# lsp-plugins/lsp-dsp-units

Measured on AMD Instinct MI355X. Metric: Msamples/sec per GPU (biquad-x8 1024ch; Convolver 65536-tap) + HBM roofline %, higher is better.
Workload: dtype f32; 1 GPU; biquad-x8 cascade (FilterBank::process), 1024 channels x 4096-sample blocks per GPU, FLT_BT_LRX_LOPASS slope 4 per-channel cutoffs, state carried across blocks; channels_per_gpu=1024, block=4096, resident_ring_blocks=16, parallelism=channel-shard x1, no collective, blocks_per_call=1657

## Files before the change

### lsp-dsp-units_amd/csrc/biquad.hip

```cpp
#include "mi_common.h"
#include "ilufs_device.h"

#include <algorithm>
#include <atomic>
#include <cmath>
#include <cstdint>
#include <cstdlib>
#include <vector>

namespace
{
    template <int L>
    struct geom
    {
        static constexpr int W      = 2 * L;
        static constexpr int TAB    = 96 + 2 * L;
        static constexpr int PITCH  = W + 4;
        static constexpr int BLOCK  = 64 * W;
        static constexpr int SG     = 128;
        static_assert(((PITCH / 4) & 1) == 1, "LDS pitch must be an odd number of 16-B slots");
        static_assert((TAB % 16) == 0, "table rows stay 64-B aligned (s_load_dwordx16)");
    };

    constexpr int TAB_PQ = 32;
    typedef float v2f  __attribute__((ext_vector_type(2)));
    typedef float v8f  __attribute__((ext_vector_type(8)));
    typedef float v16f __attribute__((ext_vector_type(16)));

    __device__ __forceinline__ v2f pk_fma(v2f a, v2f b, v2f c) { return __builtin_elementwise_fma(a, b, c); }
    __device__ __forceinline__ v2f splat(float a) { return v2f{a, a}; }
    __device__ __forceinline__ v2f mat_fma(v2f c0, v2f c1, v2f v, v2f a) { return pk_fma(c0, splat(v.x), pk_fma(c1, splat(v.y), a)); }

    template <int CTRL, int ROW_MASK>
    __device__ __forceinline__ float dpp_or(float old, float v)
    {
        return __int_as_float(__builtin_amdgcn_update_dpp(__float_as_int(old), __float_as_int(v), CTRL, ROW_MASK, 0xf, false));
    }
    template <int CTRL, int ROW_MASK>
    __device__ __forceinline__ v2f dpp_or(v2f old, v2f v) { return v2f{dpp_or<CTRL, ROW_MASK>(old.x, v.x), dpp_or<CTRL, ROW_MASK>(old.y, v.y)}; }

    template <int CTRL>
    __device__ __forceinline__ v2f dpp_zero(v2f v)
    {
        return v2f{__int_as_float(__builtin_amdgcn_update_dpp(0, __float_as_int(v.x), CTRL, 0xf, 0xf, true)),
                   __int_as_float(__builtin_amdgcn_update_dpp(0, __float_as_int(v.y), CTRL, 0xf, 0xf, true))};
    }

    constexpr int DPP_ROW_SHR1 = 0x111, DPP_ROW_SHR2 = 0x112, DPP_ROW_SHR4 = 0x114, DPP_ROW_SHR8 = 0x118;
    constexpr int DPP_WAVE_SHR1 = 0x138, DPP_ROW_BCAST15 = 0x142, DPP_ROW_BCAST31 = 0x143;

    using mi::BUFFER_DWORD3;
    using mi::CPOL_SC1;
    using mi::u32x4;
    using mi::CPOL_NT_SC1;
    template <int POL = CPOL_NT_SC1>
    __device__ __forceinline__ void store_through(__amdgpu_buffer_rsrc_t rsrc, int dword_index, float4 v)
    {
        mi::wt_store<POL>(rsrc, dword_index * 4, v);
    }

#ifndef MI_ABLATE
#define MI_ABLATE 0
#endif
#ifdef MI_BIQUAD_PROBE
    __device__ unsigned long long g_probe[4096 * 16 * 2];
    #define MI_PROBE(slot) do { __builtin_amdgcn_sched_barrier(0); if (t == 0 && (slot) < 16) { \
        const unsigned pw_ = blockIdx.x * (blockDim.x >> 6) + (threadIdx.x >> 6); \
        g_probe[(pw_ * 16 + (slot)) * 2] = wall_clock64(); \
        g_probe[(pw_ * 16 + (slot)) * 2 + 1] = __builtin_readcyclecounter(); } __builtin_amdgcn_sched_barrier(0); } while (0)
#else
    #define MI_PROBE(slot) do { } while (0)
#endif
    constexpr int CHAIN_MAX = 14;
    struct chain_stage
    {
        const float    *tab;
        float          *state;
        const uint32_t *nsec;
        float          *out;
        size_t          out_stride;
        int             max_sec;
        int             branch;
    };
    struct chain_args
// ... 83 lines not shown
        {
            for (int i = tid; i < group; i += NT)
                sstate[par][lds0 + i] = reinterpret_cast<const float2 *>(mem + size_t(s0) * 2)[i];
        };
        auto flush_state = [&](float *mem, int s0, int group, int par, int lds0)
        {
            for (int i = tid; i < group; i += NT)
                reinterpret_cast<float2 *>(mem + size_t(s0) * 2)[i] = sstate[par][lds0 + i];
        };

        v2f x[L];

        struct sectab
        {
            v16f pq[L / 8];
            v8f  m0;
            v16f m1;
            float4 cf;
            float  a2;
            float4 ql;
        };
        typedef const __attribute__((address_space(4))) float cfloat;
        auto uniform_row = [&](const float *T) -> cfloat * {
            const uint64_t v = reinterpret_cast<uint64_t>(T);
            const uint32_t lo = uint32_t(__builtin_amdgcn_readfirstlane(int(uint32_t(v))));
            const uint32_t hi = uint32_t(__builtin_amdgcn_readfirstlane(int(uint32_t(v >> 32))));
            return reinterpret_cast<cfloat *>((uint64_t(hi) << 32) | lo);
        };
        typedef const __attribute__((address_space(4))) v16f cv16f;
        typedef const __attribute__((address_space(4))) v8f cv8f;
        auto load_pq = [&](sectab &r, const float *T)
        {
            cfloat *U = uniform_row(T);
            #pragma unroll
            for (int j = 0; j < L / 8; ++j)
                r.pq[j] = *reinterpret_cast<cv16f *>(U + TAB_PQ + 16 * j);
        };
        auto load_mats = [&](sectab &r, const float *T)
        {
            cfloat *U = uniform_row(T);
            r.m0 = *reinterpret_cast<cv8f *>(U + 8);
            r.m1 = *reinterpret_cast<cv16f *>(U + 16);
            r.ql = *reinterpret_cast<const float4 *>(T + TAB_QL + 4 * l16);
        };
        auto load_coefs = [&](sectab &r, const float *T)
        {
            cfloat *U = uniform_row(T);
            r.cf = make_float4(U[0], U[1], U[2], U[3]);
            r.a2 = U[4];
        };

        auto section = [&](sectab &tb, const float *Tnext, int si, int par, bool saver, bool save_hi)
        {
            v2f a0 = splat(0.0f), a1_ = splat(0.0f), b0_ = splat(0.0f), b1_ = splat(0.0f);
            #pragma unroll
            for (int k = 0; k < L; k += 2)
            {
                const v16f &r = tb.pq[k / 8];
                const v2f pq0 = v2f{r[(2 * k) % 16], r[(2 * k + 1) % 16]};
                const v2f pq1 = v2f{r[(2 * k + 2) % 16], r[(2 * k + 3) % 16]};
                a0  = pk_fma(pq0, splat(x[k].x), a0);      b0_ = pk_fma(pq0, splat(x[k].y), b0_);
                a1_ = pk_fma(pq1, splat(x[k + 1].x), a1_); b1_ = pk_fma(pq1, splat(x[k + 1].y), b1_);
            }
            const v2f zwA = a0 + a1_, zwB = b0_ + b1_;

            const v2f Pc0 = v2f{tb.m0[0], tb.m0[1]}, Pc1 = v2f{tb.m0[2], tb.m0[3]};
            v2f e = mat_fma(Pc0, Pc1, zwA, zwB);

            if (XW > 1)
                for (int v = 0; v < wv; ++v)
                    __syncthreads();
            const float2 cs = (XW > 1 && wv > 0) ? xchg[par][si][wv - 1] : sstate[par][si];
            const v2f cvec = lane0 ? v2f{cs.x, cs.y} : splat(0.0f);
            e = mat_fma(v2f{tb.m0[4], tb.m0[5]}, v2f{tb.m0[6], tb.m0[7]}, cvec, e);

            const v2f zero = splat(0.0f);
            e = mat_fma(v2f{tb.m0[4], tb.m0[5]}, v2f{tb.m0[6], tb.m0[7]}, dpp_zero<DPP_ROW_SHR1>(e), e);
            e = mat_fma(v2f{tb.m1[0], tb.m1[1]}, v2f{tb.m1[2], tb.m1[3]}, dpp_zero<DPP_ROW_SHR2>(e), e);
            e = mat_fma(v2f{tb.m1[4], tb.m1[5]}, v2f{tb.m1[6], tb.m1[7]}, dpp_zero<DPP_ROW_SHR4>(e), e);
            e = mat_fma(v2f{tb.m1[8], tb.m1[9]}, v2f{tb.m1[10], tb.m1[11]}, dpp_zero<DPP_ROW_SHR8>(e), e);
            const v2f QLc0 = v2f{tb.ql.x, tb.ql.y}, QLc1 = v2f{tb.ql.z, tb.ql.w};
            e = mat_fma(QLc0, QLc1, dpp_or<DPP_ROW_BCAST15, 0xa>(zero, e), e);
            {
                const v2f s  = dpp_or<DPP_ROW_BCAST31, 0xc>(zero, e);
                const v2f s2 = mat_fma(v2f{tb.m1[12], tb.m1[13]}, v2f{tb.m1[14], tb.m1[15]}, s, zero);
                e = mat_fma(QLc0, QLc1, row3 ? s2 : s, e);
            }
            if (XW > 1)
            {
                if (t == 63)
                    xchg[par][si][wv] = make_float2(e.x, e.y);
                for (int v = wv; v < XW - 1; ++v)
                    __syncthreads();
            }

            const v2f S  = dpp_or<DPP_WAVE_SHR1, 0xf>(cvec, e);
            const v2f SB = mat_fma(Pc0, Pc1, S, zwA);
            v2f d0 = v2f{S.x, SB.x}, d1 = v2f{S.y, SB.y};
            __builtin_amdgcn_sched_barrier(0);
            load_pq(tb, Tnext);
            load_mats(tb, Tnext);
            __builtin_amdgcn_sched_barrier(0);

            const v2f b0 = splat(tb.cf.x), b1 = splat(tb.cf.y), b2 = splat(tb.cf.z), a1 = splat(tb.cf.w), a2 = splat(tb.a2);
            #pragma unroll
            for (int k = 0; k < L; ++k)
            {
                const v2f xx = x[k];
                const v2f tq = pk_fma(b1, xx, d1);
                const v2f u  = b2 * xx;
                const v2f y  = pk_fma(b0, xx, d0);
                d0   = pk_fma(a1, y, tq);
                d1   = pk_fma(a2, y, u);
                x[k] = y;
            }
            __builtin_amdgcn_sched_barrier(0);
            load_coefs(tb, Tnext);
// ... 348 lines not shown

#ifdef MI_BIQUAD_PROBE
    #define MI_STREAM_PROBE_BEGIN() unsigned long long pc_[4] = {0, 0, 0, 0}, pt_ = __builtin_readcyclecounter(), pw0_ = wall_clock64(), \
        pw1_ = 0, pw2_ = 0; const unsigned long long pc0_ = pt_; unsigned spins_ = 0
    #define MI_STREAM_PROBE(slot) do { __builtin_amdgcn_sched_barrier(0); const unsigned long long now_ = __builtin_readcyclecounter(); \
        pc_[slot] += now_ - pt_; pt_ = now_; if ((slot) == 1 && pw1_ == 0) pw1_ = wall_clock64(); if ((slot) == 3 && pw2_ == 0) pw2_ = wall_clock64(); \
        __builtin_amdgcn_sched_barrier(0); } while (0)
    #define MI_STREAM_PROBE_SPIN() (++spins_)
    #define MI_STREAM_PROBE_ITER(it) do { if (t == 0 && (it) < 20) g_probe[(size_t(blockIdx.x) * NW + wv) * 32 + 11 + (it)] = \
        (wall_clock64() & 0xffffffffull) | ((__builtin_readcyclecounter() & 0xffffffffull) << 32); } while (0)
    #define MI_STREAM_PROBE_END() do { if (t == 0) { unsigned long long *p_ = g_probe + (size_t(blockIdx.x) * NW + wv) * 32; \
        p_[0] = pw0_; p_[1] = wall_clock64(); p_[2] = __builtin_readcyclecounter() - pc0_; p_[3] = pc_[1]; p_[4] = pc_[2]; p_[5] = pc_[3] + pc_[0]; \
        p_[6] = spins_; p_[7] = pw1_; p_[8] = pw2_; \
        p_[9] = __builtin_amdgcn_s_getreg((31 << 11) | 4); p_[10] = __builtin_amdgcn_s_getreg((31 << 11) | 20); } } while (0)
#else
    #define MI_STREAM_PROBE_BEGIN() do { } while (0)
    #define MI_STREAM_PROBE(slot) do { } while (0)
    #define MI_STREAM_PROBE_SPIN() do { } while (0)
    #define MI_STREAM_PROBE_ITER(it) do { } while (0)
    #define MI_STREAM_PROBE_END() do { } while (0)
#endif
#ifndef MI_STREAM_ROTATE
#define MI_STREAM_ROTATE 1
#endif
    constexpr int STREAM_MAX_BLOCKS = 128;
    constexpr int STREAM_SG         = 32;
    struct stream_args
    {
        int             blocks;
        float          *out[STREAM_MAX_BLOCKS];
        const float    *in[STREAM_MAX_BLOCKS];
    };
    constexpr int STREAM_CHAIN_BLOCKS = 64;
    constexpr int STREAM_CHAIN_PTRS   = 320;
    struct stream_chain_stage
    {
        const float    *tab;
        float          *state;
        const uint32_t *nsec;
        int             max_sec;
        int             slot;
        int             branch;
    };
    struct stream_chain_args
    {
        int                 blocks, stages, outs;
        stream_chain_stage  st[CHAIN_MAX];
        const float        *in[STREAM_CHAIN_BLOCKS];
        float              *out[STREAM_CHAIN_PTRS];
    };
    struct stream_cell { float d0, d1; uint32_t seq, pad; };
    typedef volatile __attribute__((address_space(3))) stream_cell lds_cell;

    template <int NW, bool CHAIN, bool QLDS>
    __device__ __forceinline__
    void biquad_stream_body(const stream_args *pa, const stream_chain_args *pc, size_t out_stride, size_t in_stride,
                            int n , const float *__restrict__ tab, float *state,
                            const uint32_t *__restrict__ nsec, int max_sec, int cap)
    {
        using G = geom<16>;
        constexpr int L = 16, W = G::W, TAB = G::TAB, PITCH = G::PITCH, SB = G::BLOCK;
        constexpr int LPT = W / 4;
        constexpr int TAB_QL = TAB_PQ + 2 * L;
        __shared__ __attribute__((aligned(16))) float sx_all[NW * 64 * PITCH];
        extern __shared__ float4 stream_dyn[];
        stream_cell *const cell = reinterpret_cast<stream_cell *>(stream_dyn);
        const float4 *const sql = stream_dyn + cap * NW;

        const int ch  = int(blockIdx.x);
        const int tid = int(threadIdx.x);
        const int t   = tid & 63;
        const int wv  = __builtin_amdgcn_readfirstlane(tid >> 6);
        const int l16 = t & 15;
        float *const sx = sx_all + wv * 64 * PITCH;
        const bool lane0 = (t == 0), row3 = (t >= 48);
        const int nst = CHAIN ? pc->stages : 1;
        auto stage_ns  = [&](int k) -> int { return CHAIN ? int(pc->st[k].nsec[ch]) : int(nsec[ch]); };
        auto stage_tab = [&](int k) -> const float * {
            return CHAIN ? pc->st[k].tab + size_t(ch) * pc->st[k].max_sec * TAB : tab + size_t(ch) * max_sec * TAB; };
        auto stage_mem = [&](int k) -> float * {
            return CHAIN ? pc->st[k].state + size_t(ch) * pc->st[k].max_sec * 2 : state + size_t(ch) * max_sec * 2; };
        const float *ctab = stage_tab(0);
        float2 *const mem0 = reinterpret_cast<float2 *>(stage_mem(0));
        const int spb   = (n + SB - 1) / SB;
        const int total = (CHAIN ? pc->blocks : pa->blocks) * spb;
        const int pred  = (wv + NW - 1) % NW;

        typedef const __attribute__((address_space(4))) float cfloat;
        typedef const __attribute__((address_space(4))) v16f cv16f;
        typedef const __attribute__((address_space(4))) v8f cv8f;
        auto uniform_row = [&](const float *T) -> cfloat * {
            const uint64_t v = reinterpret_cast<uint64_t>(T);
            const uint32_t lo = uint32_t(__builtin_amdgcn_readfirstlane(int(uint32_t(v))));
            const uint32_t hi = uint32_t(__builtin_amdgcn_readfirstlane(int(uint32_t(v >> 32))));
            return reinterpret_cast<cfloat *>((uint64_t(hi) << 32) | lo);
        };
        struct sectab
        {
            v16f pq[L / 8];
            v8f  m0;
            v16f m1;
            float4 cf;
            float  a2;
            float4 ql;
        };
        auto load_pq = [&](sectab &r, const float *T)
        {
            cfloat *U = uniform_row(T);
            #pragma unroll
            for (int j = 0; j < L / 8; ++j)
                r.pq[j] = *reinterpret_cast<cv16f *>(U + TAB_PQ + 16 * j);
        };
        auto load_mats = [&](sectab &r, const float *T, int qi )
        {
            cfloat *U = uniform_row(T);
            r.m0 = *reinterpret_cast<cv8f *>(U + 8);
            r.m1 = *reinterpret_cast<cv16f *>(U + 16);
            r.ql = QLDS ? sql[qi * 16 + l16] : *reinterpret_cast<const float4 *>(T + TAB_QL + 4 * l16);
        };
        auto load_coefs = [&](sectab &r, const float *T)
        {
            cfloat *U = uniform_row(T);
            r.cf = make_float4(U[0], U[1], U[2], U[3]);
            r.a2 = U[4];
        };

        float4 ld[LPT];
        auto issue_loads = [&](int g, bool there = true)
        {
            const int k = g / spb, j = g - k * spb;
            const float *blk = CHAIN ? pc->in[k] : pa->in[k];
            const __amdgpu_buffer_rsrc_t src = __builtin_amdgcn_make_buffer_rsrc(
                const_cast<float *>(blk + size_t(ch) * in_stride), 0, there ? n * 4 : 0, BUFFER_DWORD3);
            #pragma unroll
            for (int q = 0; q < LPT; ++q)
            {
                const u32x4 v = __builtin_amdgcn_raw_buffer_load_b128(src, (j * SB + 4 * (q * 64 + t)) * 4, 0, 0);
                ld[q] = make_float4(__uint_as_float(v.x), __uint_as_float(v.y), __uint_as_float(v.z), __uint_as_float(v.w));
            }
        };

        if (wv < total)
            issue_loads(wv);
        if (QLDS)
        {
            const __amdgpu_buffer_rsrc_t none = __builtin_amdgcn_make_buffer_rsrc(state, 0, 0, BUFFER_DWORD3);
            #pragma unroll
            for (int q = 0; q < LPT; ++q)
                store_through(none, 4 * (q * 64 + t), make_float4(0.0f, 0.0f, 0.0f, 0.0f));
        }
        const int ns  = stage_ns(0);
        if (!CHAIN && ns < 0)
            return;
        {
            int lds0 = 0;
            for (int k = 0; k < nst; ++k)
            {
                const int nk = (k == 0) ? ns : stage_ns(k);
                const float *mk = stage_mem(k);
                for (int i = tid; i < nk * NW; i += 64 * NW)
                {
                    const int si = i / NW, w = i - si * NW;
                    stream_cell c = { 0.0f, 0.0f, 0u, 0u };
                    if (w == NW - 1)
                    {
                        const float2 s = reinterpret_cast<const float2 *>(mk)[si];
                        c.d0 = s.x;
                        c.d1 = s.y;
                    }
                    cell[(lds0 + si) * NW + w] = c;
                }
                if (QLDS)
                {
                    const float *tk = stage_tab(k);
                    for (int i = tid; i < nk * 16; i += 64 * NW)
                        stream_dyn[cap * NW + lds0 * 16 + i] = *reinterpret_cast<const float4 *>(tk + size_t(i >> 4) * TAB + TAB_QL + 4 * (i & 15));
                }
                lds0 += nk;
            }
        }
        __syncthreads();

        v2f x[L];
        sectab tb;
        if (CHAIN || ns > 0)
        {
            load_pq(tb, ctab);
            load_mats(tb, ctab, 0);
            load_coefs(tb, ctab);
        }
        MI_STREAM_PROBE_BEGIN();

        for (int g = wv; g < total; g += NW)
        {
            MI_STREAM_PROBE(0);
            const int k = g / spb, j = g - k * spb;
            const int base  = j * SB;
            const int valid = (n - base < SB) ? n - base : SB;
            const int last  = valid - 1;
            const int t_last = last / W;
            const bool save_hi = (last - t_last * W) >= L;
            const bool saver   = (t == t_last);
            const bool exact_out = (j & 1) || (j == spb - 1);
            const bool final_sb  = (g == total - 1);
            const uint32_t want = uint32_t(g), mine = uint32_t(g + 1);

            #pragma unroll
            for (int q = 0; q < LPT; ++q)
            {
                const int i = 4 * (q * 64 + t);
                float *d = &sx[(i / W) * PITCH + 2 * (i % L) + ((i % W) / L)];
                d[0] = ld[q].x; d[2] = ld[q].y; d[4] = ld[q].z; d[6] = ld[q].w;
            }
            __builtin_amdgcn_wave_barrier();
            MI_STREAM_PROBE(1);
            if (!CHAIN && g + NW < total)
                issue_loads(g + NW);
            #pragma unroll
            for (int q = 0; q < L / 2; ++q)
            {
                const float4 v = *reinterpret_cast<const float4 *>(&sx[t * PITCH + 4 * q]);
                x[2 * q] = v2f{v.x, v.y};
                x[2 * q + 1] = v2f{v.z, v.w};
            }

            auto section = [&](const float *Tnext, int qnext, int ci, float2 *mem2, int turn)
            {
#if MI_STREAM_ROTATE
                if ((turn & 3) == 0)
                    switch (((turn >> 2) + (g / NW) + int(blockIdx.x >> 8)) & 3)
                    {
                        case 0: __builtin_amdgcn_s_setprio(3); break;
                        case 1: __builtin_amdgcn_s_setprio(2); break;
                        case 2: __builtin_amdgcn_s_setprio(1); break;
                        default: __builtin_amdgcn_s_setprio(0); break;
                    }
#endif
                lds_cell *const from = (lds_cell *)&cell[ci * NW + pred];
                lds_cell *const to   = (lds_cell *)&cell[ci * NW + wv];
                uint32_t got = from->seq;
                float c0 = from->d0, c1 = from->d1;

                v2f a0 = splat(0.0f), a1_ = splat(0.0f), b0_ = splat(0.0f), b1_ = splat(0.0f);
                #pragma unroll
                for (int q = 0; q < L; q += 2)
                {
                    const v16f &r = tb.pq[q / 8];
                    const v2f pq0 = v2f{r[(2 * q) % 16], r[(2 * q + 1) % 16]};
                    const v2f pq1 = v2f{r[(2 * q + 2) % 16], r[(2 * q + 3) % 16]};
                    a0  = pk_fma(pq0, splat(x[q].x), a0);      b0_ = pk_fma(pq0, splat(x[q].y), b0_);
                    a1_ = pk_fma(pq1, splat(x[q + 1].x), a1_); b1_ = pk_fma(pq1, splat(x[q + 1].y), b1_);
                }
                const v2f zwA = a0 + a1_, zwB = b0_ + b1_;

                const v2f Pc0 = v2f{tb.m0[0], tb.m0[1]}, Pc1 = v2f{tb.m0[2], tb.m0[3]};
                v2f e = mat_fma(Pc0, Pc1, zwA, zwB);
                asm volatile("" : "+v"(e));
                while (got != want)
                {
                    MI_STREAM_PROBE_SPIN();
                    __builtin_amdgcn_s_sleep(1);
                    got = from->seq;
                    c0 = from->d0;
                    c1 = from->d1;
                }
                const v2f cvec = lane0 ? v2f{c0, c1} : splat(0.0f);
                e = mat_fma(v2f{tb.m0[4], tb.m0[5]}, v2f{tb.m0[6], tb.m0[7]}, cvec, e);

                const v2f zero = splat(0.0f);
                e = mat_fma(v2f{tb.m0[4], tb.m0[5]}, v2f{tb.m0[6], tb.m0[7]}, dpp_zero<DPP_ROW_SHR1>(e), e);
                e = mat_fma(v2f{tb.m1[0], tb.m1[1]}, v2f{tb.m1[2], tb.m1[3]}, dpp_zero<DPP_ROW_SHR2>(e), e);
                e = mat_fma(v2f{tb.m1[4], tb.m1[5]}, v2f{tb.m1[6], tb.m1[7]}, dpp_zero<DPP_ROW_SHR4>(e), e);
                e = mat_fma(v2f{tb.m1[8], tb.m1[9]}, v2f{tb.m1[10], tb.m1[11]}, dpp_zero<DPP_ROW_SHR8>(e), e);
                const v2f QLc0 = v2f{tb.ql.x, tb.ql.y}, QLc1 = v2f{tb.ql.z, tb.ql.w};
                e = mat_fma(QLc0, QLc1, dpp_or<DPP_ROW_BCAST15, 0xa>(zero, e), e);
                {
                    const v2f s  = dpp_or<DPP_ROW_BCAST31, 0xc>(zero, e);
                    const v2f s2 = mat_fma(v2f{tb.m1[12], tb.m1[13]}, v2f{tb.m1[14], tb.m1[15]}, s, zero);
                    e = mat_fma(QLc0, QLc1, row3 ? s2 : s, e);
                }
                if (!exact_out && t == 63)
                {
                    to->d0 = e.x;
                    to->d1 = e.y;
                    to->seq = mine;
                }

                const v2f S  = dpp_or<DPP_WAVE_SHR1, 0xf>(cvec, e);
                const v2f SB2 = mat_fma(Pc0, Pc1, S, zwA);
                v2f d0 = v2f{S.x, SB2.x}, d1 = v2f{S.y, SB2.y};
                __builtin_amdgcn_sched_barrier(0);
                load_pq(tb, Tnext);
                load_mats(tb, Tnext, qnext);
                __builtin_amdgcn_sched_barrier(0);

                const v2f b0 = splat(tb.cf.x), b1 = splat(tb.cf.y), b2 = splat(tb.cf.z), a1 = splat(tb.cf.w), a2 = splat(tb.a2);
                #pragma unroll
                for (int q = 0; q < L; ++q)
                {
                    const v2f xx = x[q];
                    const v2f tq = pk_fma(b1, xx, d1);
                    const v2f u  = b2 * xx;
                    const v2f y  = pk_fma(b0, xx, d0);
                    d0   = pk_fma(a1, y, tq);
                    d1   = pk_fma(a2, y, u);
                    x[q] = y;
                }
                __builtin_amdgcn_sched_barrier(0);
                load_coefs(tb, Tnext);
                if (saver && (exact_out || final_sb))
                {
                    const float s0 = save_hi ? d0.y : d0.x, s1 = save_hi ? d1.y : d1.x;
                    if (exact_out)
                    {
                        to->d0 = s0;
                        to->d1 = s1;
                        to->seq = mine;
                    }
                    if (final_sb)
                        *mem2 = make_float2(s0, s1);
                }
            };
            auto store_tile = [&](float *rows)
            {
                const __amdgpu_buffer_rsrc_t dst = __builtin_amdgcn_make_buffer_rsrc(rows + size_t(ch) * out_stride, 0, n * 4, BUFFER_DWORD3);
                #pragma unroll
                for (int q = 0; q < L / 2; ++q)
                    *reinterpret_cast<float4 *>(&sx[t * PITCH + 4 * q]) = make_float4(x[2 * q].x, x[2 * q].y, x[2 * q + 1].x, x[2 * q + 1].y);
                __builtin_amdgcn_wave_barrier();
                #pragma unroll
                for (int q = 0; q < LPT; ++q)
                {
                    const int i = 4 * (q * 64 + t);
                    const float *d = &sx[(i / W) * PITCH + 2 * (i % L) + ((i % W) / L)];
                    store_through(dst, base + i, make_float4(d[0], d[2], d[4], d[6]));
                }
                __builtin_amdgcn_wave_barrier();
            };

            if constexpr (!CHAIN)
            {
                for (int si = 0; si < ns; ++si)
                {
                    const int snext = (si + 1 < ns) ? si + 1 : 0;
                    section(ctab + size_t(snext) * TAB, snext, si, mem0 + si, si);
                }
                MI_STREAM_PROBE(2);
                store_tile(pa->out[k]);
            }
            else
            {
                struct stage_info { int ns; const float *T; float2 *mem2; int slot, branch; };
                auto fetch = [&](int q) -> stage_info {
                    stage_info v;
                    v.ns = stage_ns(q);
                    v.T = stage_tab(q);
                    v.mem2 = reinterpret_cast<float2 *>(stage_mem(q));
                    v.slot = pc->st[q].slot;
                    v.branch = pc->st[q].branch;
                    return v;
                };
                auto run_stage = [&](auto may_branch, const stage_info &cur, const float *Tn, int lds0, int qn )
                {
                    constexpr bool BR = decltype(may_branch)::value;
                    v2f xs[L];
                    if (BR && cur.branch)
                    {
                        #pragma unroll
                        for (int i = 0; i < L; ++i)
                            xs[i] = x[i];
                    }
                    for (int si = 0; si < cur.ns; ++si)
                        section((si + 1 < cur.ns) ? cur.T + size_t(si + 1) * TAB : Tn, (si + 1 < cur.ns) ? lds0 + si + 1 : qn,
                                lds0 + si, cur.mem2 + si, lds0 + si);
                    if (cur.slot >= 0)
                        store_tile(pc->out[k * pc->outs + cur.slot]);
                    if (BR && cur.branch)
                    {
                        #pragma unroll
                        for (int i = 0; i < L; ++i)
                            x[i] = xs[i];
                    }
                };
                int lds0 = 0;
                stage_info cur = fetch(0);
                for (int q = 0; q + 1 < nst; ++q)
                {
                    const stage_info nxt = fetch(q + 1);
                    run_stage(std::true_type(), cur, nxt.T, lds0, lds0 + cur.ns);
                    lds0 += cur.ns;
                    cur = nxt;
                }
                {
                    const bool more = g + NW < total;
                    issue_loads(more ? g + NW : g, more);
                }
                run_stage(std::false_type(), cur, ctab, lds0, 0);
                MI_STREAM_PROBE(2);
            }
            MI_STREAM_PROBE(3);
            MI_STREAM_PROBE_ITER(g / NW);
        }
        MI_STREAM_PROBE_END();
    }

    __device__ unsigned long long g_stream_clock[4];

    template <int NW, bool QLDS>
    __global__ __launch_bounds__(64 * NW, (NW >= 4) ? 4 : 2)
    void biquad_stream_kernel(const stream_args a, size_t out_stride, size_t in_stride, int n ,
                              const float *__restrict__ tab, float *state, const uint32_t *__restrict__ nsec, int max_sec, int cap)
    {
        const bool stamp = blockIdx.x == 0 && threadIdx.x == 0;
        if (stamp)
        {
            g_stream_clock[0] = __builtin_readcyclecounter();
            g_stream_clock[1] = wall_clock64();
        }
        biquad_stream_body<NW, false, QLDS>(&a, nullptr, out_stride, in_stride, n, tab, state, nsec, max_sec, cap);
        if (stamp)
        {
            g_stream_clock[2] = __builtin_readcyclecounter();
            g_stream_clock[3] = wall_clock64();
        }
    }

    template <int NW, bool QLDS>
    __global__ __launch_bounds__(64 * NW, 4)
    void biquad_stream_chain_kernel(const stream_chain_args c, size_t out_stride, size_t in_stride, int n , int cap)
    {
        biquad_stream_body<NW, true, QLDS>(nullptr, &c, out_stride, in_stride, n, nullptr, nullptr, nullptr, 0, cap);
    }

    inline bool stream_qlds(int nw, int cap) { return size_t(nw) * 64 * geom<16>::PITCH * 4 + size_t(cap) * (nw + 16) * 16 <= 40960; }
    inline size_t stream_lds(int nw, int cap, bool qlds) { return size_t(cap) * (nw + (qlds ? 16 : 0)) * 16; }

    __global__ void biquad_tail_kernel(float *out, const float *in, size_t out_stride, size_t in_stride,
                                       size_t start, int count , const float *__restrict__ tab, int tab_row,
                                       float *state, const uint32_t *__restrict__ nsec, int max_sec, uint32_t channels,
                                       const sumsq_args sq)
    {
        const uint32_t ch = blockIdx.x * blockDim.x + threadIdx.x;
        if (ch >= channels)
            return;
        const int ns = int(nsec[ch]);
        if (ns < 0)
            return;
        float xs[16];
        for (int k = 0; k < 16; ++k)
            xs[k] = (k < count) ? in[size_t(ch) * in_stride + start + k] : 0.0f;
        for (int s = 0; s < ns; ++s)
        {
            const float *q = tab + (size_t(ch) * max_sec + s) * tab_row;
            float *st = state + (size_t(ch) * max_sec + s) * 2;
            const float b0 = q[0], b1 = q[1], b2 = q[2], a1 = q[3], a2 = q[4];
            float d0 = st[0], d1 = st[1];
            for (int k = 0; k < count; ++k)
            {
                const float xx = xs[k];
                const float tq = fmaf(b1, xx, d1);
                const float u  = b2 * xx;
                const float y  = fmaf(b0, xx, d0);
                d0 = fmaf(a1, y, tq);
                d1 = fmaf(a2, y, u);
                xs[k] = y;
            }
            st[0] = d0;
            st[1] = d1;
        }
        if (sq.sums != nullptr)
        {
            float acc[4] = { 0.0f, 0.0f, 0.0f, 0.0f };
            for (int k = 0; k < count; ++k)
            {
                const int i = int(start) + k, sk = int(i >= sq.e0) + int(i >= sq.e1) + int(i >= sq.e2);
                for (int j = 0; j < 4; ++j)
                    acc[j] = (sk == j) ? fmaf(xs[k], xs[k], acc[j]) : acc[j];
            }
            for (int j = 0; j < 4; ++j)
                sq.sums[size_t(ch) * 4 + j] += acc[j];
            return;
        }
        for (int k = 0; k < count; ++k)
            out[size_t(ch) * out_stride + start + k] = xs[k];
    }

    __global__ __launch_bounds__(64)
    void biquad_reference_ir_kernel(float *out, size_t stride, int n, const float *__restrict__ tab, int tab_row,
// ... 492 lines not shown
            a.st[k].branch = stages[k].branch ? 1 : 0;
        }
        const bool loop = mi::test_path("blocks_loop");
        const size_t spb = (samples + big::BLOCK - 1) / big::BLOCK;
        const size_t out_bytes = (size_t(channels - 1) * out_stride + samples) * sizeof(float);
        const size_t in_bytes  = (size_t(channels - 1) * in_stride + samples) * sizeof(float);
        auto overlap = [](const void *p, size_t pn, const void *q, size_t qn) -> bool {
            const uintptr_t a0 = reinterpret_cast<uintptr_t>(p), b0 = reinterpret_cast<uintptr_t>(q);
            return a0 < b0 + qn && b0 < a0 + pn;
        };
        auto joins = [&](size_t first, size_t k) -> bool {
            if (loop)
                return false;
            for (int s = 0; s < outs; ++s)
            {
                const float *o = out[k * outs + s];
                if (o != in[k] && overlap(o, out_bytes, in[k], in_bytes))
                    return false;
                for (int q = 0; q < s; ++q)
                    if (overlap(o, out_bytes, out[k * outs + q], out_bytes))
                        return false;
            }
            for (size_t i = first; i < k; ++i)
                for (int s = 0; s < outs; ++s)
                {
                    if (overlap(out[i * outs + s], out_bytes, in[k], in_bytes) || overlap(in[i], in_bytes, out[k * outs + s], out_bytes))
                        return false;
                    for (int q = 0; q < outs; ++q)
                        if (overlap(out[i * outs + s], out_bytes, out[k * outs + q], out_bytes) &&
                            (out[i * outs + s] != out[k * outs + q] || (((k - i) * spb) % NW) != 0))
                            return false;
                }
            return true;
        };
        const size_t cap = std::min<size_t>(size_t(STREAM_CHAIN_BLOCKS), size_t(STREAM_CHAIN_PTRS) / size_t(outs));
        size_t first = 0;
        while (first < blocks)
        {
            size_t n = 0;
            while (first + n < blocks && n < cap && joins(first, first + n))
                ++n;
            if (n >= 2 || (n == 1 && spb >= 4 && !loop))
            {
                a.blocks = int(n);
                for (size_t i = 0; i < n; ++i)
                {
                    a.in[i] = in[first + i];
                    for (int s = 0; s < outs; ++s)
                        a.out[i * outs + s] = out[(first + i) * outs + s];
                }
                hipEvent_t ev0 = nullptr, ev1 = nullptr;
                take_profile_events(&ev0, &ev1);
                const int nw = (n * spb >= 4) ? 4 : 2;
                const bool qlds = stream_qlds(nw, sec_cap);
                const size_t lds = stream_lds(nw, sec_cap, qlds);
                #define MI_STREAM(NWV, Q) MI_LAUNCH((biquad_stream_chain_kernel<NWV, Q>), dim3(channels), dim3(64 * NWV), lds, st, ev0, ev1, a, \
                                                    out_stride, in_stride, int(samples), sec_cap)
                if (nw == 4) { if (qlds) MI_STREAM(4, true); else MI_STREAM(4, false); }
                else         { if (qlds) MI_STREAM(2, true); else MI_STREAM(2, false); }
                #undef MI_STREAM
                MI_HIP_CHECK(hipGetLastError());
            }
            else
            {
                n = 1;
                biquad_chain_stage one[CHAIN_MAX];
                for (int k = 0; k < count; ++k)
                {
                    one[k] = stages[k];
                    one[k].out = (slot[k] >= 0) ? out[first * outs + slot[k]] : nullptr;
                    one[k].out_stride = out_stride;
                }
                const int r = biquad_chain_process(one, count, in[first], in_stride, samples, st, false);
                if (r != MI_OK)
                    return (r == 1) ? fail(MI_ESTATE, "biquad_chain_process_blocks: a block of a qualified run was turned down") : r;
            }
            first += n;
        }
        return MI_OK;
    }
}

static int bank_run(mi_biquad_bank_t *b, float *out, const float *in, size_t samples, size_t out_stride, size_t in_stride,
                    hipStream_t st, const sumsq_args *sq, const mi_meters::ilufs_epilogue *ep = nullptr, bool *rode = nullptr);

namespace mi
{
    int biquad_bank_reference_impulse_response(mi_biquad_bank *b, float *out, size_t samples, size_t out_stride, hipStream_t st)
    {
        MI_REQUIRE(b != nullptr && out != nullptr && out_stride >= samples && samples < (size_t(1) << 29), MI_EINVAL,
                   "biquad_bank_reference_impulse_response: bad argument");
        if (samples == 0)
            return MI_OK;
        const int r = commit(b, st);
        if (r != MI_OK)
            return r;
        hipLaunchKernelGGL(biquad_reference_ir_kernel, dim3(b->channels), dim3(64), 0, st, out, out_stride, int(samples),
                           b->d_small, int(small::TAB), b->d_nsec, int(b->max_sec));
        MI_HIP_CHECK(hipGetLastError());
        return MI_OK;
    }

    void biquad_bank_output_reread(mi_biquad_bank *b, bool yes) { if (b != nullptr) b->out_reread = yes; }

    int biquad_bank_sumsq(mi_biquad_bank *b, const float *in, size_t in_stride, size_t samples, const uint32_t seg_end[3],
                          float *sums, hipStream_t st, const mi_meters::ilufs_epilogue *ep, bool *rode)
    {
        if (rode != nullptr)
            *rode = false;
        if (samples == 0)
            return MI_OK;
        MI_REQUIRE(b != nullptr && in != nullptr && sums != nullptr && in_stride >= samples && samples < (size_t(1) << 31),
// ... 271 lines not shown
                           int(b->max_sec), b->channels, sq ? *sq : sumsq_args{ nullptr, 0, 0, 0 });
        MI_HIP_CHECK(hipGetLastError());
    }
    return MI_OK;
}

int mi_biquad_bank_process(mi_biquad_bank_t *b, float *out, const float *in, size_t samples,
                           size_t out_stride, size_t in_stride, void *stream)
{
    MI_REQUIRE(b != nullptr, MI_ESTATE, "mi_biquad_bank_process: NULL bank");
    if (samples == 0)
        return MI_OK;
    MI_REQUIRE(out != nullptr && in != nullptr, MI_EINVAL, "mi_biquad_bank_process: NULL buffer");
    MI_REQUIRE(out_stride >= samples && in_stride >= samples, MI_EINVAL,
               "mi_biquad_bank_process: stride shorter than the block");
    if (samples >= 4 * size_t(big::BLOCK) && (samples % 16) == 0 && samples < (size_t(1) << 28) && (out_stride % 4) == 0 &&
        (in_stride % 4) == 0 && ((reinterpret_cast<uintptr_t>(out) | reinterpret_cast<uintptr_t>(in)) % 16) == 0 && !b->exact &&
        !mi::test_path("blocks_loop"))
    {
        bool fits = true;
        for (uint32_t c = 0; fits && c < b->channels; ++c)
            fits = b->nsec[c] <= uint32_t(STREAM_SG);
        if (fits)
        {
            const int r = commit(b, mi::as_stream(stream));
            if (r != MI_OK)
                return r;
            float *po[1] = { out };
            const float *pi[1] = { in };
            return stream_launch(b, po, pi, 0, 1, samples, out_stride, in_stride, mi::as_stream(stream));
        }
    }
    return bank_run(b, out, in, samples, out_stride, in_stride, mi::as_stream(stream), nullptr);
}

static int stream_launch(mi_biquad_bank_t *b, float *const *out, const float *const *in, size_t first, size_t count,
                         size_t samples, size_t out_stride, size_t in_stride, hipStream_t st)
{
    stream_args a;
    a.blocks = int(count);
    for (size_t k = 0; k < count; ++k)
    {
        a.out[k] = out[first + k];
        a.in[k]  = in[first + k];
    }
    const size_t subs = count * ((samples + big::BLOCK - 1) / big::BLOCK);
    const int nw = (subs >= 4) ? 4 : 2;
    const dim3 grid(b->channels);
    hipEvent_t ev0 = nullptr, ev1 = nullptr;
    mi::take_profile_events(&ev0, &ev1);
    int cap = 1;
    for (uint32_t c = 0; c < b->channels; ++c)
        cap = std::max(cap, int(b->nsec[c]));
    const bool qlds = stream_qlds(nw, cap);
    const size_t lds = stream_lds(nw, cap, qlds);
    #define MI_STREAM(NWV, Q) MI_LAUNCH((biquad_stream_kernel<NWV, Q>), grid, dim3(64 * NWV), lds, st, ev0, ev1, a, out_stride, in_stride, \
                                        int(samples), b->d_big, b->d_state, b->d_nsec, int(b->max_sec), cap)
    if (nw == 4)      { if (qlds) MI_STREAM(4, true); else MI_STREAM(4, false); }
    else if (nw == 2) { if (qlds) MI_STREAM(2, true); else MI_STREAM(2, false); }
    else              { if (qlds) MI_STREAM(2, true); else MI_STREAM(2, false); }
    #undef MI_STREAM
    MI_HIP_CHECK(hipGetLastError());
    return MI_OK;
}

int mi_biquad_bank_process_blocks(mi_biquad_bank_t *b, float *const *out, const float *const *in, size_t blocks,
                                  size_t samples, size_t out_stride, size_t in_stride, void *stream)
{
    MI_REQUIRE(b != nullptr, MI_ESTATE, "mi_biquad_bank_process_blocks: NULL bank");
    if (samples == 0 || blocks == 0)
        return MI_OK;
    MI_REQUIRE(out != nullptr && in != nullptr, MI_EINVAL, "mi_biquad_bank_process_blocks: NULL pointer table");
    MI_REQUIRE(out_stride >= samples && in_stride >= samples, MI_EINVAL,
               "mi_biquad_bank_process_blocks: stride shorter than the block");
    for (size_t k = 0; k < blocks; ++k)
        MI_REQUIRE(out[k] != nullptr && in[k] != nullptr, MI_EINVAL, "mi_biquad_bank_process_blocks: NULL buffer of block %zu", k);
    hipStream_t st = mi::as_stream(stream);
    int r = commit(b, st);
    if (r != MI_OK)
        return r;

    bool streamable = samples > 2 * size_t(small::BLOCK) && (samples % 16) == 0 && samples < (size_t(1) << 28) && !b->exact &&
                      (out_stride % 4) == 0 && (in_stride % 4) == 0 && !mi::test_path("blocks_loop");
    for (uint32_t c = 0; streamable && c < b->channels; ++c)
        streamable = b->nsec[c] <= uint32_t(STREAM_SG);
    const size_t spb = (samples + big::BLOCK - 1) / big::BLOCK;
    const size_t out_bytes = (size_t(b->channels - 1) * out_stride + samples) * sizeof(float);
    const size_t in_bytes  = (size_t(b->channels - 1) * in_stride + samples) * sizeof(float);
    auto overlap = [](const void *p, size_t pn, const void *q, size_t qn) -> bool {
        const uintptr_t a0 = reinterpret_cast<uintptr_t>(p), b0 = reinterpret_cast<uintptr_t>(q);
        return a0 < b0 + qn && b0 < a0 + pn;
    };
    auto joins = [&](size_t first, size_t k) -> bool {
        if (!streamable || ((reinterpret_cast<uintptr_t>(out[k]) | reinterpret_cast<uintptr_t>(in[k])) % 16) != 0)
            return false;
        for (size_t i = first; i < k; ++i)
        {
            if (overlap(out[i], out_bytes, in[k], in_bytes) || overlap(in[i], in_bytes, out[k], out_bytes))
                return false;
            if (overlap(out[i], out_bytes, out[k], out_bytes) && (out[i] != out[k] || (((k - i) * spb) % 4) != 0))
                return false;
        }
        return true;
    };
    size_t first = 0;
    while (first < blocks)
    {
        size_t count = 0;
        while (first + count < blocks && count < size_t(STREAM_MAX_BLOCKS) && joins(first, first + count))
            ++count;
        if (count >= 2)
            r = stream_launch(b, out, in, first, count, samples, out_stride, in_stride, st);
        else
// ... 81 lines not shown
```

Before: 596,400 Msamples/s.

## Compute chunk-end states in stream kernel with MFMA 4x4x1 from LDS weights

Moves the per-chunk end-state dot products in the streaming biquad kernel from packed VALU FMAs onto the matrix cores, using mfma_f32_4x4x1f32 with a reorganised weight table staged in LDS. The LDS layout gains a transposed weight region plus a zero pad, and a three-tier form selection picks MFMA, vector-with-LDS or plain variants according to LDS budget. It also hoists the LDS scatter/gather address computation into a single register reused across the loops. The MFMA path adds LDS footprint and latency on the scan's critical chain, and it relies on lanes beyond the first two reading zero weights.

```diff
diff --git a/lsp-dsp-units_amd/csrc/biquad.hip b/lsp-dsp-units_amd/csrc/biquad.hip
--- a/lsp-dsp-units_amd/csrc/biquad.hip
+++ b/lsp-dsp-units_amd/csrc/biquad.hip
@@ -30,6 +30,37 @@
     __device__ __forceinline__ v2f pk_fma(v2f a, v2f b, v2f c) { return __builtin_elementwise_fma(a, b, c); }
     __device__ __forceinline__ v2f splat(float a) { return v2f{a, a}; }
     __device__ __forceinline__ v2f mat_fma(v2f c0, v2f c1, v2f v, v2f a) { return pk_fma(c0, splat(v.x), pk_fma(c1, splat(v.y), a)); }
+
+    template <int L>
+    __device__ __forceinline__ void chunk_end_states(const v16f (&pq)[L / 8], const v2f (&x)[L], v2f &zwA, v2f &zwB)
+    {
+        v2f a = splat(0.0f), b = splat(0.0f);
+        #pragma unroll
+        for (int k = 0; k < L; ++k)
+        {
+            const v16f &r = pq[k / 8];
+            const v2f w = v2f{r[(2 * k) % 16], r[(2 * k + 1) % 16]};
+            a = pk_fma(w, splat(x[k].x), a);
+            b = pk_fma(w, splat(x[k].y), b);
+        }
+        zwA = a;
+        zwB = b;
+    }
+    typedef float v4f __attribute__((ext_vector_type(4)));
+    __device__ __forceinline__ void chunk_end_states_mfma(const float4 (&wt)[4], const v2f (&x)[16], v2f &zwA, v2f &zwB)
+    {
+        v4f a = v4f{0.0f, 0.0f, 0.0f, 0.0f}, b = v4f{0.0f, 0.0f, 0.0f, 0.0f};
+        #pragma unroll
+        for (int k = 0; k < 16; ++k)
+        {
+            const float4 q = wt[k / 4];
+            const float w = (k % 4 == 0) ? q.x : (k % 4 == 1) ? q.y : (k % 4 == 2) ? q.z : q.w;
+            a = __builtin_amdgcn_mfma_f32_4x4x1f32(w, x[k].x, a, 0, 0, 0);
+            b = __builtin_amdgcn_mfma_f32_4x4x1f32(w, x[k].y, b, 0, 0, 0);
+        }
+        zwA = v2f{a[0], a[1]};
+        zwB = v2f{b[0], b[1]};
+    }
 
     template <int CTRL, int ROW_MASK>
     __device__ __forceinline__ float dpp_or(float old, float v)
@@ -219,17 +250,8 @@
 
         auto section = [&](sectab &tb, const float *Tnext, int si, int par, bool saver, bool save_hi)
         {
-            v2f a0 = splat(0.0f), a1_ = splat(0.0f), b0_ = splat(0.0f), b1_ = splat(0.0f);
-            #pragma unroll
-            for (int k = 0; k < L; k += 2)
-            {
-                const v16f &r = tb.pq[k / 8];
-                const v2f pq0 = v2f{r[(2 * k) % 16], r[(2 * k + 1) % 16]};
-                const v2f pq1 = v2f{r[(2 * k + 2) % 16], r[(2 * k + 3) % 16]};
-                a0  = pk_fma(pq0, splat(x[k].x), a0);      b0_ = pk_fma(pq0, splat(x[k].y), b0_);
-                a1_ = pk_fma(pq1, splat(x[k + 1].x), a1_); b1_ = pk_fma(pq1, splat(x[k + 1].y), b1_);
-            }
-            const v2f zwA = a0 + a1_, zwB = b0_ + b1_;
+            v2f zwA, zwB;
+            chunk_end_states<L>(tb.pq, x, zwA, zwB);
 
             const v2f Pc0 = v2f{tb.m0[0], tb.m0[1]}, Pc1 = v2f{tb.m0[2], tb.m0[3]};
             v2f e = mat_fma(Pc0, Pc1, zwA, zwB);
@@ -684,7 +706,7 @@
     struct stream_cell { float d0, d1; uint32_t seq, pad; };
     typedef volatile __attribute__((address_space(3))) stream_cell lds_cell;
 
-    template <int NW, bool CHAIN, bool QLDS>
+    template <int NW, bool CHAIN, bool QLDS, bool MFMA>
     __device__ __forceinline__
     void biquad_stream_body(const stream_args *pa, const stream_chain_args *pc, size_t out_stride, size_t in_stride,
                             int n , const float *__restrict__ tab, float *state,
@@ -695,9 +717,11 @@
         constexpr int LPT = W / 4;
         constexpr int TAB_QL = TAB_PQ + 2 * L;
         __shared__ __attribute__((aligned(16))) float sx_all[NW * 64 * PITCH];
+        static_assert(QLDS || !MFMA, "the weight table follows the scan operands");
         extern __shared__ float4 stream_dyn[];
         stream_cell *const cell = reinterpret_cast<stream_cell *>(stream_dyn);
         const float4 *const sql = stream_dyn + cap * NW;
+        const float4 *const swt = sql + cap * 16;
 
         const int ch  = int(blockIdx.x);
         const int tid = int(threadIdx.x);
@@ -706,6 +730,7 @@
         const int l16 = t & 15;
         float *const sx = sx_all + wv * 64 * PITCH;
         const bool lane0 = (t == 0), row3 = (t >= 48);
+        const int wt_step = ((t & 3) < 2) ? 8 : 0, wt_first = ((t & 3) < 2) ? 4 * (t & 3) : cap * 8 + 2;
         const int nst = CHAIN ? pc->stages : 1;
         auto stage_ns  = [&](int k) -> int { return CHAIN ? int(pc->st[k].nsec[ch]) : int(nsec[ch]); };
         auto stage_tab = [&](int k) -> const float * {
@@ -756,6 +781,20 @@
             r.cf = make_float4(U[0], U[1], U[2], U[3]);
             r.a2 = U[4];
         };
+        sectab tb;
+        float4 wt[4];
+        auto load_weights = [&](const float *T, int qi)
+        {
+            if constexpr (MFMA)
+            {
+                const float4 *w = swt + qi * wt_step + wt_first;
+                #pragma unroll
+                for (int i = 0; i < 4; ++i)
+                    wt[i] = w[i];
+            }
+            else
+                load_pq(tb, T);
+        };
 
         float4 ld[LPT];
         auto issue_loads = [&](int g, bool there = true)
@@ -808,16 +847,27 @@
                     for (int i = tid; i < nk * 16; i += 64 * NW)
                         stream_dyn[cap * NW + lds0 * 16 + i] = *reinterpret_cast<const float4 *>(tk + size_t(i >> 4) * TAB + TAB_QL + 4 * (i & 15));
                 }
+                if (MFMA)
+                {
+                    const float *tk = stage_tab(k);
+                    #pragma unroll 1
+                    for (int i = tid; i < nk * 8; i += 64 * NW)
+                    {
+                        const float *r = tk + ((i >> 3) * TAB + TAB_PQ + 8 * (i & 3) + ((i >> 2) & 1));
+                        stream_dyn[cap * (NW + 16) + lds0 * 8 + i] = make_float4(r[0], r[2], r[4], r[6]);
+                    }
+                }
                 lds0 += nk;
             }
+            if (MFMA && tid < 8)
+                stream_dyn[cap * (NW + 24) + tid] = make_float4(0.0f, 0.0f, 0.0f, 0.0f);
         }
         __syncthreads();
 
         v2f x[L];
-        sectab tb;
         if (CHAIN || ns > 0)
         {
-            load_pq(tb, ctab);
+            load_weights(ctab, 0);
             load_mats(tb, ctab, 0);
             load_coefs(tb, ctab);
         }
@@ -837,11 +887,13 @@
             const bool final_sb  = (g == total - 1);
             const uint32_t want = uint32_t(g), mine = uint32_t(g + 1);
 
+            int piece0 = ((4 * t) / W) * PITCH + 2 * ((4 * t) % L) + (((4 * t) % W) / L);
+            if (MFMA)
+                asm volatile("" : "+v"(piece0));
             #pragma unroll
             for (int q = 0; q < LPT; ++q)
             {
-                const int i = 4 * (q * 64 + t);
-                float *d = &sx[(i / W) * PITCH + 2 * (i % L) + ((i % W) / L)];
+                float *d = &sx[piece0 + q * (256 / W) * PITCH];
                 d[0] = ld[q].x; d[2] = ld[q].y; d[4] = ld[q].z; d[6] = ld[q].w;
             }
             __builtin_amdgcn_wave_barrier();
@@ -873,17 +925,15 @@
                 uint32_t got = from->seq;
                 float c0 = from->d0, c1 = from->d1;
 
-                v2f a0 = splat(0.0f), a1_ = splat(0.0f), b0_ = splat(0.0f), b1_ = splat(0.0f);
-                #pragma unroll
-                for (int q = 0; q < L; q += 2)
-                {
-                    const v16f &r = tb.pq[q / 8];
-                    const v2f pq0 = v2f{r[(2 * q) % 16], r[(2 * q + 1) % 16]};
-                    const v2f pq1 = v2f{r[(2 * q + 2) % 16], r[(2 * q + 3) % 16]};
-                    a0  = pk_fma(pq0, splat(x[q].x), a0);      b0_ = pk_fma(pq0, splat(x[q].y), b0_);
-                    a1_ = pk_fma(pq1, splat(x[q + 1].x), a1_); b1_ = pk_fma(pq1, splat(x[q + 1].y), b1_);
-                }
-                const v2f zwA = a0 + a1_, zwB = b0_ + b1_;
+                v2f zwA, zwB;
+                if constexpr (MFMA)
+                {
+                    chunk_end_states_mfma(wt, x, zwA, zwB);
+                    __builtin_amdgcn_sched_group_barrier(0x100, 3, 0);
+                    __builtin_amdgcn_sched_group_barrier(0x008, 32, 0);
+                }
+                else
+                    chunk_end_states<L>(tb.pq, x, zwA, zwB);
 
                 const v2f Pc0 = v2f{tb.m0[0], tb.m0[1]}, Pc1 = v2f{tb.m0[2], tb.m0[3]};
                 v2f e = mat_fma(Pc0, Pc1, zwA, zwB);
@@ -922,7 +972,7 @@
                 const v2f SB2 = mat_fma(Pc0, Pc1, S, zwA);
                 v2f d0 = v2f{S.x, SB2.x}, d1 = v2f{S.y, SB2.y};
                 __builtin_amdgcn_sched_barrier(0);
-                load_pq(tb, Tnext);
+                load_weights(Tnext, qnext);
                 load_mats(tb, Tnext, qnext);
                 __builtin_amdgcn_sched_barrier(0);
 
@@ -960,11 +1010,14 @@
                 for (int q = 0; q < L / 2; ++q)
                     *reinterpret_cast<float4 *>(&sx[t * PITCH + 4 * q]) = make_float4(x[2 * q].x, x[2 * q].y, x[2 * q + 1].x, x[2 * q + 1].y);
                 __builtin_amdgcn_wave_barrier();
+                int piece = piece0;
+                if (MFMA)
+                    asm volatile("" : "+v"(piece));
                 #pragma unroll
                 for (int q = 0; q < LPT; ++q)
                 {
                     const int i = 4 * (q * 64 + t);
-                    const float *d = &sx[(i / W) * PITCH + 2 * (i % L) + ((i % W) / L)];
+                    const float *d = &sx[piece + q * (256 / W) * PITCH];
                     store_through(dst, base + i, make_float4(d[0], d[2], d[4], d[6]));
                 }
                 __builtin_amdgcn_wave_barrier();
@@ -1049,7 +1102,7 @@
             g_stream_clock[0] = __builtin_readcyclecounter();
             g_stream_clock[1] = wall_clock64();
         }
-        biquad_stream_body<NW, false, QLDS>(&a, nullptr, out_stride, in_stride, n, tab, state, nsec, max_sec, cap);
+        biquad_stream_body<NW, false, QLDS, QLDS>(&a, nullptr, out_stride, in_stride, n, tab, state, nsec, max_sec, cap);
         if (stamp)
         {
             g_stream_clock[2] = __builtin_readcyclecounter();
@@ -1061,11 +1114,37 @@
     __global__ __launch_bounds__(64 * NW, 4)
     void biquad_stream_chain_kernel(const stream_chain_args c, size_t out_stride, size_t in_stride, int n , int cap)
     {
-        biquad_stream_body<NW, true, QLDS>(nullptr, &c, out_stride, in_stride, n, nullptr, nullptr, nullptr, 0, cap);
-    }
-
-    inline bool stream_qlds(int nw, int cap) { return size_t(nw) * 64 * geom<16>::PITCH * 4 + size_t(cap) * (nw + 16) * 16 <= 40960; }
-    inline size_t stream_lds(int nw, int cap, bool qlds) { return size_t(cap) * (nw + (qlds ? 16 : 0)) * 16; }
+        biquad_stream_body<NW, true, QLDS, QLDS>(nullptr, &c, out_stride, in_stride, n, nullptr, nullptr, nullptr, 0, cap);
+    }
+
+    template <int NW>
+    __global__ __launch_bounds__(64 * NW, (NW >= 4) ? 4 : 2)
+    void biquad_stream_vector_kernel(const stream_args a, size_t out_stride, size_t in_stride, int n ,
+                                     const float *__restrict__ tab, float *state, const uint32_t *__restrict__ nsec, int max_sec, int cap)
+    {
+        biquad_stream_body<NW, false, true, false>(&a, nullptr, out_stride, in_stride, n, tab, state, nsec, max_sec, cap);
+    }
+    template <int NW>
+    __global__ __launch_bounds__(64 * NW, 4)
+    void biquad_stream_vector_chain_kernel(const stream_chain_args c, size_t out_stride, size_t in_stride, int n , int cap)
+    {
+        biquad_stream_body<NW, true, true, false>(nullptr, &c, out_stride, in_stride, n, nullptr, nullptr, nullptr, 0, cap);
+    }
+
+    inline size_t stream_lds(int nw, int cap, int form)
+    {
+        return size_t(cap) * (nw + (form >= 1 ? 16 : 0) + (form >= 2 ? 8 : 0)) * 16 + (form >= 2 ? 128 : 0);
+    }
+    inline int stream_form(int nw, int cap)
+    {
+        const size_t tiles = size_t(nw) * 64 * geom<16>::PITCH * 4;
+        int form = 2;
+        while (form > 0 && tiles + stream_lds(nw, cap, form) > 40960)
+            --form;
+        if (form == 2 && mi::test_path("biquad_vector"))
+            form = 1;
+        return form;
+    }
 
     __global__ void biquad_tail_kernel(float *out, const float *in, size_t out_stride, size_t in_stride,
                                        size_t start, int count , const float *__restrict__ tab, int tab_row,
@@ -1664,12 +1743,14 @@
                 hipEvent_t ev0 = nullptr, ev1 = nullptr;
                 take_profile_events(&ev0, &ev1);
                 const int nw = (n * spb >= 4) ? 4 : 2;
-                const bool qlds = stream_qlds(nw, sec_cap);
-                const size_t lds = stream_lds(nw, sec_cap, qlds);
-                #define MI_STREAM(NWV, Q) MI_LAUNCH((biquad_stream_chain_kernel<NWV, Q>), dim3(channels), dim3(64 * NWV), lds, st, ev0, ev1, a, \
+                const int form = stream_form(nw, sec_cap);
+                const size_t lds = stream_lds(nw, sec_cap, form);
+                #define MI_STREAM(...) MI_LAUNCH((__VA_ARGS__), dim3(channels), dim3(64 * nw), lds, st, ev0, ev1, a, \
                                                     out_stride, in_stride, int(samples), sec_cap)
-                if (nw == 4) { if (qlds) MI_STREAM(4, true); else MI_STREAM(4, false); }
-                else         { if (qlds) MI_STREAM(2, true); else MI_STREAM(2, false); }
+                if (nw == 4) { if (form == 2) MI_STREAM(biquad_stream_chain_kernel<4, true>); else if (form == 1) MI_STREAM(biquad_stream_vector_chain_kernel<4>);
+                               else MI_STREAM(biquad_stream_chain_kernel<4, false>); }
+                else         { if (form == 2) MI_STREAM(biquad_stream_chain_kernel<2, true>); else if (form == 1) MI_STREAM(biquad_stream_vector_chain_kernel<2>);
+                               else MI_STREAM(biquad_stream_chain_kernel<2, false>); }
                 #undef MI_STREAM
                 MI_HIP_CHECK(hipGetLastError());
             }
@@ -2047,13 +2128,14 @@
     int cap = 1;
     for (uint32_t c = 0; c < b->channels; ++c)
         cap = std::max(cap, int(b->nsec[c]));
-    const bool qlds = stream_qlds(nw, cap);
-    const size_t lds = stream_lds(nw, cap, qlds);
-    #define MI_STREAM(NWV, Q) MI_LAUNCH((biquad_stream_kernel<NWV, Q>), grid, dim3(64 * NWV), lds, st, ev0, ev1, a, out_stride, in_stride, \
+    const int form = stream_form(nw, cap);
+    const size_t lds = stream_lds(nw, cap, form);
+    #define MI_STREAM(...) MI_LAUNCH((__VA_ARGS__), grid, dim3(64 * nw), lds, st, ev0, ev1, a, out_stride, in_stride, \
                                         int(samples), b->d_big, b->d_state, b->d_nsec, int(b->max_sec), cap)
-    if (nw == 4)      { if (qlds) MI_STREAM(4, true); else MI_STREAM(4, false); }
-    else if (nw == 2) { if (qlds) MI_STREAM(2, true); else MI_STREAM(2, false); }
-    else              { if (qlds) MI_STREAM(2, true); else MI_STREAM(2, false); }
+    if (nw == 4) { if (form == 2) MI_STREAM(biquad_stream_kernel<4, true>); else if (form == 1) MI_STREAM(biquad_stream_vector_kernel<4>);
+                   else MI_STREAM(biquad_stream_kernel<4, false>); }
+    else         { if (form == 2) MI_STREAM(biquad_stream_kernel<2, true>); else if (form == 1) MI_STREAM(biquad_stream_vector_kernel<2>);
+                   else MI_STREAM(biquad_stream_kernel<2, false>); }
     #undef MI_STREAM
     MI_HIP_CHECK(hipGetLastError());
     return MI_OK;
```

Measured after the change: 520,600 Msamples/s. -12.7%, worse.
